# araffin/srl-zoo

Measured on AMD Instinct MI355X. Metric: images/sec (224x224x3) AE+VAE train step, higher is better.
Workload: dtype f32; 1 GPU; synthetic 224x224x3 obs, --losses autoencoder, custom_cnn, state-dim 200, bs=256 per GPU (512 frames fwd+bwd per step per GPU), Adam lr 0.005, normalised fp32 observations resident in HBM; global_batch=256, parallelism=dp1, rccl_ranks=1, devices=1

## Files before the change

### include/srlz.h

```cpp
#ifndef SRLZ_H
#define SRLZ_H

#include <stddef.h>
#include <stdint.h>

#ifdef __cplusplus
extern "C" {
#endif

typedef void* srlz_stream_t;

enum srlz_status {
  SRLZ_OK = 0,
  SRLZ_ERR_BAD_DESC = -1,
  SRLZ_ERR_WORKSPACE = -2,
  SRLZ_ERR_HIP = -3,
  SRLZ_ERR_NULL = -4
};

#define SRLZ_ABI_VERSION 104
int srlz_version(void);
const char* srlz_last_error(void);
int srlz_device_cus(void);

// ... 429 lines not shown
int srlz_beam_search(const float* states, const float* wf, const float* bf, const float* w1, const float* b1, const float* w2,
                     const float* b2, const float* w3, const float* b3, int* best_plan, float* best_return, int* leaf_plans,
                     float* leaf_returns, void* ws, size_t ws_bytes, int N, int W, int T, int S, int A, int H, int n_rewards,
                     float gamma, const float* goal, long long goal_env_stride, float goal_weight, int goal_mode,
                     srlz_stream_t stream);

int srlz_horizon_supported(int S, int A, int H, int n_rewards, int has_reward);
int srlz_horizon_rows(const float* states, const int* actions, const int* starts, const int* len, const float* wf, const float* bf,
                      const float* w1, const float* b1, const float* w2, const float* b2, const float* w3, const float* b3, float* err,
                      float* base, float* reward_logits, float* trajectory, int N, int M, int T, int S, int A, int H, int n_rewards,
                      srlz_stream_t stream);
int srlz_horizon_sums(const float* err, const float* base, const float* reward_logits, const int* labels, const int* starts,
                      const int* len, int M, int T, long long* count, double* sum_err, double* sum_base, long long* hits,
                      srlz_stream_t stream);

int srlz_conv64_debug_program(const srlz_conv64_desc* d, int backward_data, int* out, int cap);
int srlz_linear_debug_route(int op, int M, int N, int K, int Kout, const void* a, const void* b, int has_ws, size_t ws_bytes,
                            int out[3]);
int srlz_debug_mfma_peak(float* out, int blocks, int iters, srlz_stream_t stream);
int srlz_debug_mfma_valu(float* out, int blocks, int iters, int valu_per_mfma, int kind, int split, srlz_stream_t stream);
int srlz_debug_placement(unsigned* out, int blocks, int lds_bytes, int spin, srlz_stream_t stream);
int srlz_debug_conv1_fwd_generic(const float* x_nchw, const float* w_ref, float* y_nhwc, float* stats_partial,
                                 const srlz_skinny_desc* d, srlz_stream_t stream);
int srlz_debug_conv1_fwd_u8_generic(const uint8_t* x_u8, const float* norm_lut, const float* w_ref, float* y_nhwc,
                                    float* stats_partial, const srlz_skinny_desc* d, srlz_stream_t stream);
int srlz_debug_conv1_bwd_weight_fused_generic(const float* x_nchw, const float* y_nhwc, const float* bnp, const uint8_t* argmax,
                                              const float* dpooled, const float* sums, int training, float* dw_ref, void* ws,
                                              size_t ws_bytes, const srlz_skinny_desc* d, const struct srlz_pool_desc_s* pd,
                                              srlz_stream_t stream);
int srlz_debug_conv1_bwd_weight_fused_u8_generic(const uint8_t* x_u8, const float* norm_lut, const float* y_nhwc, const float* bnp,
                                                 const uint8_t* argmax, const float* dpooled, const float* sums, int training,
                                                 float* dw_ref, void* ws, size_t ws_bytes, const srlz_skinny_desc* d,
                                                 const struct srlz_pool_desc_s* pd, srlz_stream_t stream);

#ifdef __cplusplus
}
#endif
#endif
```

### srl-zoo_amd/csrc/wino.hip

```cpp
#include "common.h"

namespace {

typedef float f32x2 __attribute__((ext_vector_type(2)));
typedef unsigned u32x2 __attribute__((ext_vector_type(2)));

constexpr int WN_THREADS = 256;
constexpr int WN_TP = 32;
constexpr int WN_CHUNK = 16 * 4 * 64 * 4;
constexpr int WN_VCHUNK = 16 * 4 * WN_TP * 4;
constexpr int WN_VCOMP = 4 * WN_TP * 4;
constexpr unsigned WN_DROP = 0x80000000u;

struct WinoProg {
  int N, G;
  int H, W;
  int PA, PB;
  int ppi, ppg, tpg;
  unsigned mPPI, mPB;
  int sPPI, sPB;
  long long gstride;
};

__global__ void conv64_wino_pack_kernel(const float* __restrict__ w_ref, float* __restrict__ uf, float* __restrict__ ub) {
// ... 93 lines not shown
#pragma unroll
  for (int hv = 0; hv < 2; ++hv) {
    f32x2 e[4][2];
#pragma unroll
    for (int r = 0; r < 4; ++r) {
      if (hv == 0) {
        e[r][0] = rw.d[r * 4 + 0] - rw.d[r * 4 + 2];
        e[r][1] = rw.d[r * 4 + 1] + rw.d[r * 4 + 2];
      } else {
        e[r][0] = rw.d[r * 4 + 2] - rw.d[r * 4 + 1];
        e[r][1] = rw.d[r * 4 + 1] - rw.d[r * 4 + 3];
      }
    }
#pragma unroll
    for (int j = 0; j < 2; ++j) {
      const int nu = 2 * hv + j;
      *(f32x2*)(Vw + (0 * 4 + nu) * WN_VCOMP) = e[0][j] - e[2][j];
      *(f32x2*)(Vw + (1 * 4 + nu) * WN_VCOMP) = e[1][j] + e[2][j];
      *(f32x2*)(Vw + (2 * 4 + nu) * WN_VCOMP) = e[2][j] - e[1][j];
      *(f32x2*)(Vw + (3 * 4 + nu) * WN_VCOMP) = e[1][j] - e[3][j];
    }
    __builtin_amdgcn_sched_barrier(0);
  }
}

__device__ __forceinline__ f32x4 wn_load4(__amdgpu_buffer_rsrc_t b, unsigned voff, int soff) {
  const __attribute__((ext_vector_type(4))) unsigned v = __builtin_amdgcn_raw_buffer_load_b128(b, voff, soff, 0);
  return f32x4{__uint_as_float(v[0]), __uint_as_float(v[1]), __uint_as_float(v[2]), __uint_as_float(v[3])};
}

constexpr int WN_AQ = 4;
static_assert(64 % WN_AQ == 0, "the ring of weight operands wraps with the tile");

__device__ __forceinline__ f32x4 wn_uload(__amdgpu_buffer_rsrc_t ub, unsigned uvoff, int step, int uo) {
  const __attribute__((ext_vector_type(4))) unsigned v = __builtin_amdgcn_raw_buffer_load_b128(ub, uvoff, (step & 63) * 4096 + uo, 0);
  return f32x4{__uint_as_float(v[0]), __uint_as_float(v[1]), __uint_as_float(v[2]), __uint_as_float(v[3])};
}

template <int PH>
__device__ __forceinline__ void wn_mfma_phase(f32x4 (&acc)[16][2], f32x4 (&aq)[WN_AQ], const float* __restrict__ Bp,
                                              __amdgpu_buffer_rsrc_t ub, unsigned uvoff, int uo) {
  f32x4 b0n = *(const f32x4*)(Bp), b1n = *(const f32x4*)(Bp + 256);
#pragma unroll
  for (int comp = 0; comp < 16; ++comp) {
    const int step = PH * 16 + comp;
    const f32x4 a = aq[step % WN_AQ];
    const f32x4 b0 = b0n, b1 = b1n;
    if (comp < 15) {
      b0n = *(const f32x4*)(Bp + (comp + 1) * WN_VCOMP);
      b1n = *(const f32x4*)(Bp + (comp + 1) * WN_VCOMP + 256);
    }
#pragma unroll
    for (int i = 0; i < 4; ++i) {
      if (PH == 0 && i == 0) {
        const f32x4 z = {0.f, 0.f, 0.f, 0.f};
        acc[comp][0] = __builtin_amdgcn_mfma_f32_16x16x4f32(a[i], b0[i], z, 0, 0, 0);
        acc[comp][1] = __builtin_amdgcn_mfma_f32_16x16x4f32(a[i], b1[i], z, 0, 0, 0);
      } else {
        acc[comp][0] = __builtin_amdgcn_mfma_f32_16x16x4f32(a[i], b0[i], acc[comp][0], 0, 0, 0);
        acc[comp][1] = __builtin_amdgcn_mfma_f32_16x16x4f32(a[i], b1[i], acc[comp][1], 0, 0, 0);
      }
    }
    aq[step % WN_AQ] = wn_uload(ub, uvoff, step + WN_AQ, uo);
  }
  __builtin_amdgcn_sched_group_barrier(0x100, 2, 0);
#pragma unroll
  for (int comp = 0; comp < 16; ++comp) {
    if (comp < 15) __builtin_amdgcn_sched_group_barrier(0x100, 2, 0);
    __builtin_amdgcn_sched_group_barrier(0x008, 8, 0);
    __builtin_amdgcn_sched_group_barrier(0x020, 1, 0);
  }
  __builtin_amdgcn_sched_barrier(0);
}

__device__ __forceinline__ float wn_row16_sum(float v) {
  v += __uint_as_float(__builtin_amdgcn_update_dpp(0, __float_as_uint(v), 0x128, 0xf, 0xf, false));
  v += __uint_as_float(__builtin_amdgcn_update_dpp(0, __float_as_uint(v), 0x124, 0xf, 0xf, false));
  v += __uint_as_float(__builtin_amdgcn_update_dpp(0, __float_as_uint(v), 0x122, 0xf, 0xf, false));
  v += __uint_as_float(__builtin_amdgcn_update_dpp(0, __float_as_uint(v), 0x121, 0xf, 0xf, false));
  return v;
}

constexpr int WN_ZBLOCKS = 64;
__global__ __launch_bounds__(256) void conv64_wino_poolsum_zero_scale_kernel(const float* __restrict__ dx, const PoolSum ps, float* __restrict__ partial,
                                                                            int N, int H, int W, long long gstride, int rows, int first_row) {
  const int g = blockIdx.y;
  const float* __restrict__ rec = ps.bnp + g * 256;
  const int c4 = threadIdx.x & 15;
  const auto [mean, pinv, psc, psh] = load_bn_quads(rec, c4);
  unsigned zmask = 0;
#pragma unroll
  for (int j = 0; j < 4; ++j) zmask |= ((fabsf(psc[j]) <= 1e-3f * fabsf(psh[j]) || psc[j] == 0.f) ? 1u : 0u) << j;
  double s1[4] = {0.0, 0.0, 0.0, 0.0}, s2[4] = {0.0, 0.0, 0.0, 0.0};
  if (__syncthreads_or(zmask != 0)) {
    const long long pixels = (long long)N * H * W;
    for (long long pix = (long long)blockIdx.x * 16 + (threadIdx.x >> 4); pix < pixels; pix += (long long)gridDim.x * 16) {
      if (!zmask) continue;
      const int n = (int)(pix / (H * W));
      const int yy = (int)(pix - (long long)n * H * W) / W, xx = (int)(pix - ((long long)n * H + yy) * W);
      const uint32_t packed = *(const uint32_t*)(ps.argmax + (size_t)g * gstride + (size_t)pix * 64 + c4 * 4);
      const f32x4 v = *(const f32x4*)(dx + (size_t)g * gstride + (size_t)pix * 64 + c4 * 4);
#pragma unroll
      for (int j = 0; j < 4; ++j)
        if ((zmask >> j) & 1u) {
          const int a = (packed >> (8 * j)) & 0xff;
          const int iy = yy * 2 - ps.pad + a / 3, ix = xx * 2 - ps.pad + a % 3;
          const float vy = ps.y[g * ps.y_gstride + ((size_t)(n * ps.H + iy) * ps.W + ix) * 64 + c4 * 4 + j];
          if (vy * psc[j] + psh[j] > 0.f) {
            s1[j] += (double)v[j];
            s2[j] += (double)(v[j] * ((vy - mean[j]) * pinv[j]));
          }
        }
    }
  }
  bn_bwd_combine_store(s1, s2, partial + ((size_t)g * rows + first_row + blockIdx.x) * 128);
}

template <bool PSUM, bool FUSE>
__global__ __launch_bounds__(WN_THREADS, 2) void conv64_wino_kernel(const float* __restrict__ x_all, const float* __restrict__ upack,
                                                                    const float* __restrict__ bias, float* __restrict__ y_all,
                                                                    float* __restrict__ stats_partial, const WinoProg P, int ntiles,
                                                                    const PoolSum ps, const float* __restrict__ x_bnp) {
  extern __shared__ __attribute__((aligned(16))) unsigned char smem[];
  float* Vs = (float*)smem;
  int* ptab = (int*)(Vs + 2 * WN_VCHUNK);

  const int tid = threadIdx.x;
  int lane = tid & 63;
  asm volatile("" : "+v"(lane));
  const int wave = tid >> 6;
  const int t_pt = wave * 8 + (lane >> 3), t_cp = lane & 7;
  const int cb = wave;
  const int l15 = lane & 15, g = lane >> 4;
  float* Vw = Vs + (t_pt * 4 + ((t_cp >> 1) ^ (((t_pt >> 2) & 1) << 1))) * 4 + 2 * (t_cp & 1);
  const float* Bp = Vs + (l15 * 4 + (g ^ (((l15 >> 2) & 1) << 1))) * 4;
  const unsigned uvoff = (unsigned)(g * 64 + 16 * cb + l15) * 16u;
  const __amdgpu_buffer_rsrc_t ub = raw_buffer(upack, 4u * WN_CHUNK * 4u);

  const int xcd = blockIdx.x & 7, wi = blockIdx.x >> 3, wpx = gridDim.x >> 3;
  const int tq = ntiles >> 3, tr = ntiles & 7;
  const int tbase = (xcd < tr) ? xcd * (tq + 1) : tr * (tq + 1) + (xcd - tr) * tq;
  const int tcnt = tq + (xcd < tr ? 1 : 0);
  int k = wi;
  if (k >= tcnt) return;

  const unsigned xbytes = (unsigned)(P.gstride * 4) + (unsigned)(P.W + 1) * 256u;
  const unsigned ybytes = (unsigned)(P.gstride * 4);
  const __amdgpu_buffer_rsrc_t sbuf = raw_buffer(stats_partial, stats_partial ? (unsigned)(P.G * (P.tpg + (PSUM ? WN_ZBLOCKS : 0))) * 512u : 0u);

  WinoRaw rw;
  WinoPatch wp;
  f32x4 aq[WN_AQ];
  int parity = 0;
  {
    const int tile = tbase + k;
    const int grp = tile / P.tpg;
    const __amdgpu_buffer_rsrc_t xb = raw_buffer(x_all + grp * P.gstride - (P.W + 1) * 64, xbytes);
    wn_patch(wp, P, tile - grp * P.tpg, t_pt, t_cp, ptab + t_pt);
    const float* bnrec = FUSE ? x_bnp + grp * 256 : nullptr;
    wn_request<FUSE>(rw, wp, xb, P.W, 0, bnrec, t_cp);
    wn_land<FUSE>(rw, wp, Vw);
    wn_request<FUSE>(rw, wp, xb, P.W, 1, bnrec, t_cp);
#pragma unroll
    for (int i = 0; i < WN_AQ; ++i) aq[i] = wn_uload(ub, uvoff, i, 0);
  }
  for (; k < tcnt; k += wpx, parity ^= 1) {
    const int tile = tbase + k;
    const int grp = tile / P.tpg;
    const int til = tile - grp * P.tpg;
    const __amdgpu_buffer_rsrc_t xb = raw_buffer(x_all + grp * P.gstride - (P.W + 1) * 64, xbytes);
    const int k2 = k + wpx;
    const bool more = k2 < tcnt;
    const int tile2 = tbase + (more ? k2 : k);
    const int grp2 = tile2 / P.tpg;
    const __amdgpu_buffer_rsrc_t xb2 = raw_buffer(x_all + grp2 * P.gstride - (P.W + 1) * 64, xbytes);
    int uo = 0;
    asm volatile("" : "+s"(uo));
    f32x4 acc[16][2];
#pragma unroll
    for (int p = 0; p < 4; ++p) {
      __syncthreads();
      wn_land<FUSE>(rw, wp, Vw + ((p + 1) & 1) * WN_VCHUNK);
      if (p < 2) {
        wn_request<FUSE>(rw, wp, xb, P.W, p + 2, FUSE ? x_bnp + grp * 256 : nullptr, t_cp);
      } else {
        if (p == 2) wn_patch(wp, P, tile2 - grp2 * P.tpg, t_pt, t_cp, ptab + (parity ^ 1) * WN_TP + t_pt);
        wn_request<FUSE>(rw, wp, xb2, P.W, p - 2, FUSE ? x_bnp + grp2 * 256 : nullptr, t_cp);
      }
      __builtin_amdgcn_sched_barrier(0);
      if (p == 0) wn_mfma_phase<0>(acc, aq, Bp, ub, uvoff, uo);
      if (p == 1) wn_mfma_phase<1>(acc, aq, Bp + WN_VCHUNK, ub, uvoff, uo);
      if (p == 2) wn_mfma_phase<2>(acc, aq, Bp, ub, uvoff, uo);
      if (p == 3) wn_mfma_phase<3>(acc, aq, Bp + WN_VCHUNK, ub, uvoff, uo);
    }
    const __amdgpu_buffer_rsrc_t yb = raw_buffer(y_all + grp * P.gstride, ybytes);
    f32x4 s4 = {0.f, 0.f, 0.f, 0.f}, q4 = {0.f, 0.f, 0.f, 0.f};
    f32x4 bias4 = {0.f, 0.f, 0.f, 0.f};
    if (bias) bias4 = *(const f32x4*)(bias + 16 * cb + 4 * g);
    f32x4 pA = {0.f, 0.f, 0.f, 0.f}, pB = pA, pthr = pA;
    const __amdgpu_buffer_rsrc_t zb = raw_buffer(PSUM ? ps.pooled + grp * P.gstride : nullptr, PSUM ? ybytes : 0u);
    if constexpr (PSUM) {
      const float* __restrict__ rec = ps.bnp + grp * 256 + 16 * cb + 4 * g;
      const f32x4 mean = *(const f32x4*)rec, pinv = *(const f32x4*)(rec + 64), psc = *(const f32x4*)(rec + 128), psh = *(const f32x4*)(rec + 192);
#pragma unroll
      for (int e = 0; e < 4; ++e) {
        const bool zero = fabsf(psc[e]) <= 1e-3f * fabsf(psh[e]) || psc[e] == 0.f;
        pthr[e] = zero ? __builtin_inff() : 0.f;
        const float isc = zero ? 0.f : 1.f / psc[e];
        pA[e] = pinv[e] * isc;
        pB[e] = zero ? 0.f : -(psh[e] * isc + mean[e]) * pinv[e];
      }
    }
#pragma unroll
    for (int s = 0; s < 2; ++s) {
      const int pix = ptab[parity * WN_TP + 16 * s + l15];
      const bool ok = pix >= 0;
      const unsigned yoff = ok ? (unsigned)pix * 256u + (unsigned)(16 * cb + 4 * g) * 4u : WN_DROP;
      f32x4 z00, z01, z10, z11;
      if constexpr (PSUM) {
        z00 = wn_load4(zb, yoff, 0); z01 = wn_load4(zb, yoff, 256);
        z10 = wn_load4(zb, yoff, P.W * 256); z11 = wn_load4(zb, yoff, P.W * 256 + 256);
      }
      const f32x4 bz = {ok ? bias4[0] : 0.f, ok ? bias4[1] : 0.f, ok ? bias4[2] : 0.f, ok ? bias4[3] : 0.f};
      f32x4 y00 = bz, y01 = bz, y10 = bz, y11 = bz;
#pragma unroll
      for (int nu = 0; nu < 4; ++nu) {
        const f32x4 t0 = acc[0 + nu][s] + acc[4 + nu][s] + acc[8 + nu][s];
        const f32x4 t1 = acc[4 + nu][s] - acc[8 + nu][s] - acc[12 + nu][s];
        if (nu < 3) { y00 += t0; y10 += t1; }
        if (nu == 1) { y01 += t0; y11 += t1; }
        if (nu >= 2) { y01 -= t0; y11 -= t1; }
      }
      __builtin_amdgcn_raw_buffer_store_b128(y00, yb, yoff, 0, 0);
      __builtin_amdgcn_raw_buffer_store_b128(y01, yb, yoff, 256, 0);
      __builtin_amdgcn_raw_buffer_store_b128(y10, yb, yoff, P.W * 256, 0);
      __builtin_amdgcn_raw_buffer_store_b128(y11, yb, yoff, P.W * 256 + 256, 0);
      if constexpr (PSUM) {
#pragma unroll
        for (int e = 0; e < 4; ++e) {
          s4[e] += ((z00[e] > pthr[e] ? y00[e] : 0.f) + (z01[e] > pthr[e] ? y01[e] : 0.f)) +
                   ((z10[e] > pthr[e] ? y10[e] : 0.f) + (z11[e] > pthr[e] ? y11[e] : 0.f));
        }
        q4 += (y00 * z00 + y01 * z01) + (y10 * z10 + y11 * z11);
      } else if constexpr (FUSE) {
        const f32x4 ts = (y00 + y01) + (y10 + y11), tq = (y00 * y00 + y01 * y01) + (y10 * y10 + y11 * y11);
#pragma unroll
        for (int e = 0; e < 4; ++e) { s4[e] += ok ? ts[e] : 0.f; q4[e] += ok ? tq[e] : 0.f; }
      } else {
        s4 += (y00 + y01) + (y10 + y11);
        q4 += (y00 * y00 + y01 * y01) + (y10 * y10 + y11 * y11);
      }
      __builtin_amdgcn_sched_barrier(0);
    }
    if constexpr (PSUM) {
#pragma unroll
      for (int e = 0; e < 4; ++e) q4[e] = __builtin_fmaf(pA[e], q4[e], pB[e] * s4[e]);
    }
#pragma unroll
    for (int e = 0; e < 4; ++e) { s4[e] = wn_row16_sum(s4[e]); q4[e] = wn_row16_sum(q4[e]); }
    const unsigned rec = (unsigned)(grp * (P.tpg + (PSUM ? WN_ZBLOCKS : 0)) + til) * 512u + (unsigned)(16 * cb + 4 * g) * 4u;
    __builtin_amdgcn_raw_buffer_store_b128(s4, sbuf, l15 == 0 ? rec : WN_DROP, 0, 0);
    __builtin_amdgcn_raw_buffer_store_b128(q4, sbuf, l15 == 0 ? rec + 256u : WN_DROP, 0, 0);
  }
}

int wino_program(WinoProg* P, const srlz_conv64_desc* d) {
  if (!d || d->transposed || d->ksize != 3 || d->stride != 1 || d->pad != 1) return 1;
  if (d->hi != d->ho || d->wi != d->wo || (d->hi & 1) || (d->wi & 1) || d->hi < 4 || d->wi < 4 || d->n <= 0) return 1;
  const int G = d->groups > 1 ? d->groups : 1;
  if (d->n % G) return 1;
  P->G = G; P->N = d->n / G; P->H = d->hi; P->W = d->wi; P->PA = d->hi / 2; P->PB = d->wi / 2;
  const long long ppi = (long long)P->PA * P->PB, ppg = ppi * P->N;
  const long long gfl = (long long)P->N * P->H * P->W * 64;
  if (gfl * 4 + (long long)(P->W + 1) * 256 >= 0x7FFF0000LL || ppg + WN_TP >= (1LL << 31) || ppi < 2) return 1;
  P->ppi = (int)ppi; P->ppg = (int)ppg; P->tpg = (int)((ppg + WN_TP - 1) / WN_TP);
  P->gstride = gfl;
  fastdiv_init((unsigned)P->ppi, &P->mPPI, &P->sPPI);
  fastdiv_init((unsigned)P->PB, &P->mPB, &P->sPB);
  return 0;
}

constexpr int WG_SP = 8;
constexpr int WG_OP = 8 * WG_SP * 64;
constexpr int WG_COMP = WG_SP * 64;

struct WinoWgradRaw { f32x2 d[12]; f32x2 g[4]; };

struct WinoWgradProg {
  int N, H, W, PA, PB, ppi;
  int total;
  int stages;
  int spw;
  unsigned mPPI, mPB;
  int sPPI, sPB;
};

// ... 232 lines not shown
  P->stages = (int)((total + WG_SP - 1) / WG_SP);
  P->mPPI = F.mPPI; P->sPPI = F.sPPI; P->mPB = F.mPB; P->sPB = F.sPB;
  int g = 2 * srlz_device_cus();
  g = (g + 15) & ~15;
  while (g > 16 && (g >> 1) * 4 > P->stages) g -= 16;
  const int slices = g >> 1;
  P->spw = (P->stages + slices - 1) / slices;
  *grid = g;
  return 0;
}

}

extern "C" int srlz_conv64_wino_supported(const srlz_conv64_desc* d) {
  WinoProg P;
  return wino_program(&P, d) ? 0 : 1;
}

extern "C" size_t srlz_conv64_wino_packed_floats(void) { return (size_t)4 * WN_CHUNK; }

extern "C" int srlz_conv64_wino_pack_weights(const float* w_ref, float* upack_fwd, float* upack_bwd, srlz_stream_t stream) {
  SRLZ_REQUIRE(w_ref && (upack_fwd || upack_bwd), SRLZ_ERR_NULL, "conv64_wino_pack_weights: null pointer");
  SRLZ_LAUNCH(conv64_wino_pack_kernel, dim3(16), dim3(256), 0, as_stream(stream), w_ref, upack_fwd, upack_bwd);
  return 0;
}

extern "C" int srlz_conv64_wino_tiles(const srlz_conv64_desc* d) {
  WinoProg P;
  if (wino_program(&P, d)) return -1;
  return P.G * P.tpg;
}

static int wino_launch(const float* x, const float* upack, const float* bias, float* y, float* partial, const WinoProg& P,
                       const PoolSum* ps, const float* x_bnp, srlz_stream_t stream) {
  const int ntiles = P.G * P.tpg;
  int grid = 2 * srlz_device_cus();
  if (ntiles < grid) grid = ntiles;
  grid = (grid + 7) & ~7;
  const size_t lds = (size_t)2 * WN_VCHUNK * 4 + 2 * WN_TP * 4;
  const PoolSum none = SRLZ_NO_POOLSUM;
  hipStream_t st = as_stream(stream);
  if (ps) {
    SRLZ_MAX_LDS((conv64_wino_kernel<true, false>), lds);
    SRLZ_LAUNCH((conv64_wino_kernel<true, false>), dim3(grid), dim3(WN_THREADS), lds, st, x, upack, bias, y, partial, P, ntiles, *ps, x_bnp);
  } else if (x_bnp) {
    SRLZ_MAX_LDS((conv64_wino_kernel<false, true>), lds);
    SRLZ_LAUNCH((conv64_wino_kernel<false, true>), dim3(grid), dim3(WN_THREADS), lds, st, x, upack, bias, y, partial, P, ntiles, none, x_bnp);
  } else {
    SRLZ_MAX_LDS((conv64_wino_kernel<false, false>), lds);
    SRLZ_LAUNCH((conv64_wino_kernel<false, false>), dim3(grid), dim3(WN_THREADS), lds, st, x, upack, bias, y, partial, P, ntiles, none, x_bnp);
  }
  if (ps) {
    SRLZ_LAUNCH(conv64_wino_poolsum_zero_scale_kernel, dim3(WN_ZBLOCKS, P.G), dim3(256), 0, st, (const float*)y, *ps, partial, P.N, P.H,
                P.W, P.gstride, P.tpg + WN_ZBLOCKS, P.tpg);
  }
  return 0;
}

extern "C" int srlz_conv64_wino_bwd_data_rows(const srlz_conv64_desc* d) {
  WinoProg P;
  if (wino_program(&P, d)) return -1;
  return P.G * (P.tpg + WN_ZBLOCKS);
}

extern "C" int srlz_conv64_wino_fwd(const float* x, const float* upack, const float* bias, float* y, float* stats_partial,
                                    const float* x_bnp, const srlz_conv64_desc* d, srlz_stream_t stream) {
  SRLZ_REQUIRE(x && upack && y, SRLZ_ERR_NULL, "conv64_wino_fwd: null pointer");
  WinoProg P;
  SRLZ_REQUIRE(wino_program(&P, d) == 0, SRLZ_ERR_BAD_DESC,
               "conv64_wino_fwd: 3x3 stride 1 pad 1 on even sizes only (ask srlz_conv64_wino_supported)");
  return wino_launch(x, upack, bias, y, stats_partial, P, nullptr, x_bnp, stream);
}

extern "C" int srlz_conv64_wino_bwd_data(const float* dy, const float* upack_bwd, float* dx, const srlz_conv64_desc* d, srlz_stream_t stream) {
  SRLZ_REQUIRE(dy && upack_bwd && dx, SRLZ_ERR_NULL, "conv64_wino_bwd_data: null pointer");
  WinoProg P;
  SRLZ_REQUIRE(wino_program(&P, d) == 0, SRLZ_ERR_BAD_DESC,
               "conv64_wino_bwd_data: 3x3 stride 1 pad 1 on even sizes only (ask srlz_conv64_wino_supported)");
  return wino_launch(dy, upack_bwd, nullptr, dx, nullptr, P, nullptr, nullptr, stream);
}

extern "C" int srlz_conv64_wino_bwd_data_pool_sums(const float* dy, const float* upack_bwd, float* dx, const float* pooled,
                                                   const float* pool_bnp, const float* pool_y, const uint8_t* pool_argmax,
                                                   const srlz_pool_desc* pd, float* bn_bwd_partial, const srlz_conv64_desc* d,
                                                   srlz_stream_t stream) {
  SRLZ_REQUIRE(dy && upack_bwd && dx && pooled && pool_bnp && pool_y && pool_argmax && pd && bn_bwd_partial, SRLZ_ERR_NULL,
               "conv64_wino_bwd_data_pool_sums: null pointer");
  WinoProg P;
  SRLZ_REQUIRE(wino_program(&P, d) == 0, SRLZ_ERR_BAD_DESC,
               "conv64_wino_bwd_data_pool_sums: 3x3 stride 1 pad 1 on even sizes only (ask srlz_conv64_wino_supported)");
  SRLZ_REQUIRE(pd->n == d->n && pd->hp == d->hi && pd->wp == d->wi && !pd->out_nchw && (pd->groups > 1 ? pd->groups : 1) == P.G,
               SRLZ_ERR_BAD_DESC, "conv64_wino_bwd_data_pool_sums: the pooled map [%d,%d,%d] is not this layer's input [%d,%d,%d]", pd->n, pd->hp,
               pd->wp, d->n, d->hi, d->wi);
  const PoolSum ps = {pooled, pool_bnp, pool_y, pool_argmax, (long long)(pd->n / P.G) * pd->h * pd->w * 64, pd->h, pd->w, pd->pool_pad};
  return wino_launch(dy, upack_bwd, nullptr, dx, bn_bwd_partial, P, &ps, nullptr, stream);
}

extern "C" size_t srlz_conv64_wino_bwd_weight_workspace(const srlz_conv64_desc* d) {
  WinoWgradProg P;
  int grid;
  if (wino_wgrad_program(&P, d, &grid)) return 0;
  return (size_t)grid * 8 * 4096 * sizeof(float) + (size_t)WG_CHUNKS * 16 * 4096 * sizeof(double);
}

extern "C" int srlz_conv64_wino_bwd_weight(const float* x, const float* dy, float* dw_ref, void* ws, size_t ws_bytes,
                                           const srlz_conv64_desc* d, srlz_stream_t stream) {
  SRLZ_REQUIRE(x && dy && dw_ref && ws, SRLZ_ERR_NULL, "conv64_wino_bwd_weight: null pointer");
  WinoWgradProg P;
  int grid;
  SRLZ_REQUIRE(wino_wgrad_program(&P, d, &grid) == 0, SRLZ_ERR_BAD_DESC,
               "conv64_wino_bwd_weight: 3x3 stride 1 pad 1 on even sizes only (ask srlz_conv64_wino_supported)");
  const size_t part_bytes = (size_t)grid * 8 * 4096 * sizeof(float);
  SRLZ_REQUIRE(ws_bytes >= part_bytes + (size_t)WG_CHUNKS * 16 * 4096 * sizeof(double), SRLZ_ERR_WORKSPACE,
               "conv64_wino_bwd_weight: workspace too small (%zu bytes)", ws_bytes);
  hipStream_t st = as_stream(stream);
  const size_t lds = (size_t)4 * WG_OP * 4;
  SRLZ_MAX_LDS(conv64_wino_wgrad_kernel, lds);
  SRLZ_LAUNCH(conv64_wino_wgrad_kernel, dim3(grid), dim3(256), lds, st, x, dy, (float*)ws, P);
  double* mid = (double*)((char*)ws + part_bytes);
  const int npair = grid >> 1, per = (npair + WG_CHUNKS - 1) / WG_CHUNKS;
  SRLZ_LAUNCH(conv64_wino_wgrad_reduce_a, dim3(65536 / 256, WG_CHUNKS), dim3(256), 0, st, (const float*)ws, mid, grid, per);
  SRLZ_LAUNCH(conv64_wino_wgrad_reduce_b, dim3(256), dim3(256), 0, st, (const double*)mid, WG_CHUNKS, dw_ref);
  return 0;
}
```

### srl-zoo_amd/srlz/_cabi.py

```python
import ctypes
import os
from ctypes import c_int, c_longlong, c_ulonglong, c_float, c_double, c_void_p, c_size_t, c_char_p, POINTER, Structure

_HERE = os.path.dirname(os.path.abspath(__file__))
LIB_PATH = os.path.join(_HERE, "libsrlz_hip.so")


ABI_VERSION = 104


class SrlzError(RuntimeError):
    pass


class Conv64Desc(Structure):
    _fields_ = [("n", c_int), ("hi", c_int), ("wi", c_int), ("ho", c_int), ("wo", c_int), ("ksize", c_int),
                ("stride", c_int), ("pad", c_int), ("transposed", c_int), ("groups", c_int)]


class SkinnyDesc(Structure):
    _fields_ = [("n", c_int), ("c", c_int), ("himg", c_int), ("wimg", c_int), ("hf", c_int), ("wf", c_int),
                ("kind", c_int), ("groups", c_int)]


# ... 47 lines not shown
_ID = POINTER(InferDecDesc)

_PROTOS = {
    "srlz_version": (c_int, []),
    "srlz_last_error": (c_char_p, []),
    "srlz_device_cus": (c_int, []),
    "srlz_conv64_packed_floats": (c_size_t, []),
    "srlz_conv64_pack_weights": (c_int, [P, P, P, _C64, P]),
    "srlz_conv64_fwd_tiles": (c_int, [_C64]),
    "srlz_conv64_fwd": (c_int, [P, P, P, P, P, P, _C64, P]),
    "srlz_conv64_bwd_data": (c_int, [P, P, P, _BO, _C64, P]),
    "srlz_conv64_bwd_weight_workspace": (c_size_t, [_C64]),
    "srlz_conv64_bwd_fused_supported": (c_int, [_C64]),
    "srlz_conv64_gather_pipe_supported": (c_int, [_C64, c_int]),
    "srlz_conv64_scatter_pipe_supported": (c_int, [_C64, c_int]),
    "srlz_conv64_bwd_fused_workspace": (c_size_t, [_C64]),
    "srlz_conv64_bwd_fused": (c_int, [P, P, P, _BO, P, P, P, P, P, P, c_size_t, _C64, P]),
    "srlz_conv64_bwd_fused_bn_rows": (c_int, [_C64]),
    "srlz_conv64_wino_supported": (c_int, [_C64]),
    "srlz_conv64_wino_packed_floats": (c_size_t, []),
    "srlz_conv64_wino_pack_weights": (c_int, [P, P, P, P]),
    "srlz_conv64_wino_tiles": (c_int, [_C64]),
    "srlz_conv64_wino_fwd": (c_int, [P, P, P, P, P, P, _C64, P]),
    "srlz_conv64_wino_bwd_data": (c_int, [P, P, P, _C64, P]),
    "srlz_conv64_wino_bwd_weight_workspace": (c_size_t, [_C64]),
    "srlz_conv64_wino_bwd_weight": (c_int, [P, P, P, P, c_size_t, _C64, P]),
    "srlz_conv64_wino_bwd_data_rows": (c_int, [_C64]),
    "srlz_conv64_wino_bwd_data_pool_sums": (c_int, [P, P, P, P, P, P, P, _PD, P, _C64, P]),
    "srlz_conv64_bwd_weight": (c_int, [P, P, P, P, P, _BO, P, c_size_t, _C64, P]),
    "srlz_conv64_bwd_weight_plan": (c_int, [_C64, c_int, c_int, POINTER(c_int)]),
    "srlz_conv64_bwd_fused_workgroups": (c_int, [_C64]),
    "srlz_conv1_workgroups": (c_int, [_SK]),
    "srlz_conv1_buffer_staging_supported": (c_int, [_SK]),
    "srlz_debug_conv1_fwd_generic": (c_int, [P, P, P, P, _SK, P]),
    "srlz_debug_conv1_fwd_u8_generic": (c_int, [P, P, P, P, P, _SK, P]),
    "srlz_debug_conv1_bwd_weight_fused_generic": (c_int, [P, P, P, P, P, P, c_int, P, P, c_size_t, _SK, _PD, P]),
    "srlz_debug_conv1_bwd_weight_fused_u8_generic": (c_int, [P, P, P, P, P, P, P, c_int, P, P, c_size_t, _SK, _PD, P]),
    "srlz_convT_out_os_plan": (c_int, [_SK, c_int, POINTER(c_int)]),
    "srlz_conv64_debug_program": (c_int, [_C64, c_int, POINTER(c_int), c_int]),
    "srlz_linear_debug_route": (c_int, [c_int, c_int, c_int, c_int, c_int, P, P, c_int, c_size_t, POINTER(c_int)]),
    "srlz_debug_placement": (c_int, [P, c_int, c_int, c_int, P]),
    "srlz_debug_mfma_peak": (c_int, [P, c_int, c_int, P]),
    "srlz_debug_mfma_valu": (c_int, [P, c_int, c_int, c_int, c_int, c_int, P]),
    "srlz_convn_packed_floats": (c_size_t, [_CN]),
    "srlz_convn_pack_weights": (c_int, [P, P, _CN, P]),
    "srlz_convn_fwd_tiles": (c_int, [_CN]),
    "srlz_convn_fwd": (c_int, [P, P, P, P, P, _CN, P]),
    "srlz_bn_finalize_chunks_workspace": (c_size_t, [c_int, c_int]),
    "srlz_bn_finalize_chunks": (c_int, [P, c_int, c_int, c_int, c_longlong, P, P, c_float, c_float, P, P, P, P, P, c_size_t, P]),
    "srlz_bn_eval_params_chunks": (c_int, [P, P, P, P, c_float, c_int, P, P]),
    "srlz_bn_add_relu": (c_int, [P, P, P, P, P, c_longlong, c_int, c_int, P]),
    "srlz_avgpool_nhwc": (c_int, [P, P, c_int, c_int, c_int, P]),
    "srlz_prelu_fwd": (c_int, [P, P, P, c_longlong, P]),
    "srlz_prelu_bwd": (c_int, [P, P, P, P, P, c_longlong, P]),
    "srlz_triplet_fwd": (c_int, [P, P, P, c_int, c_int, c_float, P, P, P]),
    "srlz_triplet_bwd": (c_int, [P, P, P, P, P, c_int, c_int, P, P, P, P]),
    "srlz_skinny_tiles": (c_int, [_SK]),
    "srlz_conv64_bwd_data_tiles": (c_int, [_C64]),
    "srlz_conv64_bwd_data_pool_sums": (c_int, [P, P, P, P, P, P, P, _PD, P, _C64, P]),
    "srlz_conv1_fwd": (c_int, [P, P, P, P, _SK, P]),
    "srlz_conv1_fwd_u8": (c_int, [P, P, P, P, P, _SK, P]),
    "srlz_conv1_bwd_weight_fused_u8": (c_int, [P, P, P, P, P, P, P, c_int, P, P, c_size_t, _SK, _PD, P]),
    "srlz_convT_out_fwd_loss_u8": (c_int, [P, P, P, P, P, P, P, P, P, _SK, P]),
    "srlz_normalize_lut": (c_int, [P, P]),
    "srlz_normalize_u8_planar": (c_int, [P, P, P, c_int, c_int, c_longlong, P]),
    "srlz_copy_frames_u8": (c_int, [P, P, c_longlong, P, P, c_longlong, c_int, c_longlong, P]),
# ... 222 lines not shown
```

Before: 45890 images/s.

## Fold Winograd output transform into last MFMA phase of pooled data-gradient kernel

For the pooled-sum backward-data Winograd kernel, the last matrix phase now visits components column by column and applies the output transform for each column as soon as it completes. The pooled-map loads are issued mid-phase, so the transform arithmetic and memory latency overlap the remaining MFMAs instead of running in a serial epilogue. Per-group BN pool parameters are now computed once into LDS rather than per tile. The old epilogue path stays reachable through a debug entry point, at the cost of extra LDS and register pressure in the folded kernel.

```diff
diff --git a/include/srlz.h b/include/srlz.h
--- a/include/srlz.h
+++ b/include/srlz.h
@@ -485,6 +485,10 @@
                                                  const uint8_t* argmax, const float* dpooled, const float* sums, int training,
                                                  float* dw_ref, void* ws, size_t ws_bytes, const srlz_skinny_desc* d,
                                                  const struct srlz_pool_desc_s* pd, srlz_stream_t stream);
+int srlz_debug_conv64_wino_bwd_data_pool_sums_parent(const float* dy, const float* upack_bwd, float* dx, const float* pooled,
+                                                     const float* pool_bnp, const float* pool_y, const uint8_t* pool_argmax,
+                                                     const struct srlz_pool_desc_s* pd, float* bn_bwd_partial,
+                                                     const srlz_conv64_desc* d, srlz_stream_t stream);
 
 #ifdef __cplusplus
 }
diff --git a/srl-zoo_amd/csrc/wino.hip b/srl-zoo_amd/csrc/wino.hip
--- a/srl-zoo_amd/csrc/wino.hip
+++ b/srl-zoo_amd/csrc/wino.hip
@@ -149,44 +149,92 @@
 constexpr int WN_AQ = 4;
 static_assert(64 % WN_AQ == 0, "the ring of weight operands wraps with the tile");
 
+template <bool FOLD>
+__device__ __forceinline__ constexpr int wn_comp(int ph, int i) { return (FOLD && ph == 3) ? 4 * (i & 3) + (i >> 2) : i; }
+template <bool FOLD>
+__device__ __forceinline__ constexpr int wn_step(int q) { return (q & 63) < 48 ? (q & 63) : 48 + wn_comp<FOLD>(3, q & 15); }
+
 __device__ __forceinline__ f32x4 wn_uload(__amdgpu_buffer_rsrc_t ub, unsigned uvoff, int step, int uo) {
   const __attribute__((ext_vector_type(4))) unsigned v = __builtin_amdgcn_raw_buffer_load_b128(ub, uvoff, (step & 63) * 4096 + uo, 0);
   return f32x4{__uint_as_float(v[0]), __uint_as_float(v[1]), __uint_as_float(v[2]), __uint_as_float(v[3])};
 }
 
-template <int PH>
+struct WinoFold {
+  f32x4 y[2][4];
+  f32x4 z[2][4];
+  unsigned yoff[2];
+  __amdgpu_buffer_rsrc_t zb;
+  int wrow;
+};
+
+__device__ __forceinline__ void wn_zrequest(WinoFold& f, int s) {
+  f.z[s][0] = wn_load4(f.zb, f.yoff[s], 0);
+  f.z[s][1] = wn_load4(f.zb, f.yoff[s], 256);
+  f.z[s][2] = wn_load4(f.zb, f.yoff[s], f.wrow);
+  f.z[s][3] = wn_load4(f.zb, f.yoff[s], f.wrow + 256);
+}
+
+template <int NU>
+__device__ __forceinline__ void wn_fold_column(const f32x4 (&acc)[16][2], WinoFold& f) {
+#pragma unroll
+  for (int s = 0; s < 2; ++s) {
+    const f32x4 t0 = acc[0 + NU][s] + acc[4 + NU][s] + acc[8 + NU][s];
+    const f32x4 t1 = acc[4 + NU][s] - acc[8 + NU][s] - acc[12 + NU][s];
+    if (NU < 3) { f.y[s][0] += t0; f.y[s][2] += t1; }
+    if (NU == 1) { f.y[s][1] += t0; f.y[s][3] += t1; }
+    if (NU >= 2) { f.y[s][1] -= t0; f.y[s][3] -= t1; }
+  }
+}
+
+template <int PH, bool FOLD = false>
 __device__ __forceinline__ void wn_mfma_phase(f32x4 (&acc)[16][2], f32x4 (&aq)[WN_AQ], const float* __restrict__ Bp,
-                                              __amdgpu_buffer_rsrc_t ub, unsigned uvoff, int uo) {
+                                              __amdgpu_buffer_rsrc_t ub, unsigned uvoff, int uo, WinoFold* fo = nullptr) {
+  constexpr bool CM = FOLD && PH == 3;
   f32x4 b0n = *(const f32x4*)(Bp), b1n = *(const f32x4*)(Bp + 256);
 #pragma unroll
-  for (int comp = 0; comp < 16; ++comp) {
-    const int step = PH * 16 + comp;
-    const f32x4 a = aq[step % WN_AQ];
+  for (int i = 0; i < 16; ++i) {
+    const int q = PH * 16 + i, comp = wn_comp<FOLD>(PH, i);
+    const f32x4 a = aq[q % WN_AQ];
     const f32x4 b0 = b0n, b1 = b1n;
-    if (comp < 15) {
-      b0n = *(const f32x4*)(Bp + (comp + 1) * WN_VCOMP);
-      b1n = *(const f32x4*)(Bp + (comp + 1) * WN_VCOMP + 256);
-    }
-#pragma unroll
-    for (int i = 0; i < 4; ++i) {
-      if (PH == 0 && i == 0) {
+    if (i < 15) {
+      b0n = *(const f32x4*)(Bp + wn_comp<FOLD>(PH, i + 1) * WN_VCOMP);
+      b1n = *(const f32x4*)(Bp + wn_comp<FOLD>(PH, i + 1) * WN_VCOMP + 256);
+    }
+#pragma unroll
+    for (int k = 0; k < 4; ++k) {
+      if (PH == 0 && k == 0) {
         const f32x4 z = {0.f, 0.f, 0.f, 0.f};
-        acc[comp][0] = __builtin_amdgcn_mfma_f32_16x16x4f32(a[i], b0[i], z, 0, 0, 0);
-        acc[comp][1] = __builtin_amdgcn_mfma_f32_16x16x4f32(a[i], b1[i], z, 0, 0, 0);
+        acc[comp][0] = __builtin_amdgcn_mfma_f32_16x16x4f32(a[k], b0[k], z, 0, 0, 0);
+        acc[comp][1] = __builtin_amdgcn_mfma_f32_16x16x4f32(a[k], b1[k], z, 0, 0, 0);
       } else {
-        acc[comp][0] = __builtin_amdgcn_mfma_f32_16x16x4f32(a[i], b0[i], acc[comp][0], 0, 0, 0);
-        acc[comp][1] = __builtin_amdgcn_mfma_f32_16x16x4f32(a[i], b1[i], acc[comp][1], 0, 0, 0);
-      }
-    }
-    aq[step % WN_AQ] = wn_uload(ub, uvoff, step + WN_AQ, uo);
+        acc[comp][0] = __builtin_amdgcn_mfma_f32_16x16x4f32(a[k], b0[k], acc[comp][0], 0, 0, 0);
+        acc[comp][1] = __builtin_amdgcn_mfma_f32_16x16x4f32(a[k], b1[k], acc[comp][1], 0, 0, 0);
+      }
+    }
+    aq[q % WN_AQ] = wn_uload(ub, uvoff, wn_step<FOLD>(q + WN_AQ), uo);
+    if constexpr (CM) {
+      if (i == 3) wn_fold_column<0>(acc, *fo);
+      if (i == 7) {
+        wn_fold_column<1>(acc, *fo);
+        wn_zrequest(*fo, 0);
+        wn_zrequest(*fo, 1);
+      }
+      if (i == 11) wn_fold_column<2>(acc, *fo);
+      if (i == 15) wn_fold_column<3>(acc, *fo);
+    }
   }
   __builtin_amdgcn_sched_group_barrier(0x100, 2, 0);
 #pragma unroll
-  for (int comp = 0; comp < 16; ++comp) {
-    if (comp < 15) __builtin_amdgcn_sched_group_barrier(0x100, 2, 0);
+  for (int i = 0; i < 16; ++i) {
+    if (i < 15) __builtin_amdgcn_sched_group_barrier(0x100, 2, 0);
     __builtin_amdgcn_sched_group_barrier(0x008, 8, 0);
     __builtin_amdgcn_sched_group_barrier(0x020, 1, 0);
-  }
+    if constexpr (CM) {
+      if (i == 4 || i == 8 || i == 12) __builtin_amdgcn_sched_group_barrier(0x002, 64, 0);
+      if (i == 8) __builtin_amdgcn_sched_group_barrier(0x020, 8, 0);
+    }
+  }
+  if constexpr (CM) __builtin_amdgcn_sched_group_barrier(0x002, 64, 0);
   __builtin_amdgcn_sched_barrier(0);
 }
 
@@ -233,14 +281,15 @@
   bn_bwd_combine_store(s1, s2, partial + ((size_t)g * rows + first_row + blockIdx.x) * 128);
 }
 
-template <bool PSUM, bool FUSE>
-__global__ __launch_bounds__(WN_THREADS, 2) void conv64_wino_kernel(const float* __restrict__ x_all, const float* __restrict__ upack,
-                                                                    const float* __restrict__ bias, float* __restrict__ y_all,
-                                                                    float* __restrict__ stats_partial, const WinoProg P, int ntiles,
-                                                                    const PoolSum ps, const float* __restrict__ x_bnp) {
+template <bool PSUM, bool FUSE, bool FOLD>
+__device__ __forceinline__ void wn_tiles(const float* __restrict__ x_all, const float* __restrict__ upack, const float* __restrict__ bias,
+                                         float* __restrict__ y_all, float* __restrict__ stats_partial, const WinoProg P, int ntiles,
+                                         const PoolSum ps, const float* __restrict__ x_bnp) {
+  static_assert(!FOLD || (PSUM && !FUSE), "the fold inside the matrix phase is the pooled-block data gradient's");
   extern __shared__ __attribute__((aligned(16))) unsigned char smem[];
   float* Vs = (float*)smem;
   int* ptab = (int*)(Vs + 2 * WN_VCHUNK);
+  float* pprm = (float*)(ptab + 2 * WN_TP);
 
   const int tid = threadIdx.x;
   int lane = tid & 63;
@@ -268,7 +317,7 @@
   WinoRaw rw;
   WinoPatch wp;
   f32x4 aq[WN_AQ];
-  int parity = 0;
+  int parity = 0, pgrp = -1;
   {
     const int tile = tbase + k;
     const int grp = tile / P.tpg;
@@ -294,6 +343,7 @@
     int uo = 0;
     asm volatile("" : "+s"(uo));
     f32x4 acc[16][2];
+    WinoFold fo;
 #pragma unroll
     for (int p = 0; p < 4; ++p) {
       __syncthreads();
@@ -304,11 +354,36 @@
         if (p == 2) wn_patch(wp, P, tile2 - grp2 * P.tpg, t_pt, t_cp, ptab + (parity ^ 1) * WN_TP + t_pt);
         wn_request<FUSE>(rw, wp, xb2, P.W, p - 2, FUSE ? x_bnp + grp2 * 256 : nullptr, t_cp);
       }
+      if constexpr (FOLD) {
+        if (p == 0 && grp != pgrp) {
+          pgrp = grp;
+          if (tid < 64) {
+            const float* __restrict__ rec = ps.bnp + grp * 256 + tid;
+            const float mean = rec[0], pinv = rec[64], psc = rec[128], psh = rec[192];
+            const bool zero = fabsf(psc) <= 1e-3f * fabsf(psh) || psc == 0.f;
+            const float isc = zero ? 0.f : 1.f / psc;
+            pprm[tid] = pinv * isc;
+            pprm[64 + tid] = zero ? 0.f : -__builtin_fmaf(psh, isc, mean) * pinv;
+            pprm[128 + tid] = zero ? __builtin_inff() : 0.f;
+          }
+        }
+        if (p == 3) {
+          fo.zb = raw_buffer(ps.pooled + grp * P.gstride, (unsigned)(P.gstride * 4));
+          fo.wrow = P.W * 256;
+#pragma unroll
+          for (int s = 0; s < 2; ++s) {
+            const int pix = ptab[parity * WN_TP + 16 * s + l15];
+            fo.yoff[s] = pix >= 0 ? (unsigned)pix * 256u + (unsigned)(16 * cb + 4 * g) * 4u : WN_DROP;
+#pragma unroll
+            for (int j = 0; j < 4; ++j) fo.y[s][j] = f32x4{0.f, 0.f, 0.f, 0.f};
+          }
+        }
+      }
       __builtin_amdgcn_sched_barrier(0);
-      if (p == 0) wn_mfma_phase<0>(acc, aq, Bp, ub, uvoff, uo);
-      if (p == 1) wn_mfma_phase<1>(acc, aq, Bp + WN_VCHUNK, ub, uvoff, uo);
-      if (p == 2) wn_mfma_phase<2>(acc, aq, Bp, ub, uvoff, uo);
-      if (p == 3) wn_mfma_phase<3>(acc, aq, Bp + WN_VCHUNK, ub, uvoff, uo);
+      if (p == 0) wn_mfma_phase<0, FOLD>(acc, aq, Bp, ub, uvoff, uo);
+      if (p == 1) wn_mfma_phase<1, FOLD>(acc, aq, Bp + WN_VCHUNK, ub, uvoff, uo);
+      if (p == 2) wn_mfma_phase<2, FOLD>(acc, aq, Bp, ub, uvoff, uo);
+      if (p == 3) wn_mfma_phase<3, FOLD>(acc, aq, Bp + WN_VCHUNK, ub, uvoff, uo, &fo);
     }
     const __amdgpu_buffer_rsrc_t yb = raw_buffer(y_all + grp * P.gstride, ybytes);
     f32x4 s4 = {0.f, 0.f, 0.f, 0.f}, q4 = {0.f, 0.f, 0.f, 0.f};
@@ -316,58 +391,82 @@
     if (bias) bias4 = *(const f32x4*)(bias + 16 * cb + 4 * g);
     f32x4 pA = {0.f, 0.f, 0.f, 0.f}, pB = pA, pthr = pA;
     const __amdgpu_buffer_rsrc_t zb = raw_buffer(PSUM ? ps.pooled + grp * P.gstride : nullptr, PSUM ? ybytes : 0u);
-    if constexpr (PSUM) {
-      const float* __restrict__ rec = ps.bnp + grp * 256 + 16 * cb + 4 * g;
-      const f32x4 mean = *(const f32x4*)rec, pinv = *(const f32x4*)(rec + 64), psc = *(const f32x4*)(rec + 128), psh = *(const f32x4*)(rec + 192);
-#pragma unroll
-      for (int e = 0; e < 4; ++e) {
-        const bool zero = fabsf(psc[e]) <= 1e-3f * fabsf(psh[e]) || psc[e] == 0.f;
-        pthr[e] = zero ? __builtin_inff() : 0.f;
-        const float isc = zero ? 0.f : 1.f / psc[e];
-        pA[e] = pinv[e] * isc;
-        pB[e] = zero ? 0.f : -(psh[e] * isc + mean[e]) * pinv[e];
-      }
-    }
-#pragma unroll
-    for (int s = 0; s < 2; ++s) {
-      const int pix = ptab[parity * WN_TP + 16 * s + l15];
-      const bool ok = pix >= 0;
-      const unsigned yoff = ok ? (unsigned)pix * 256u + (unsigned)(16 * cb + 4 * g) * 4u : WN_DROP;
-      f32x4 z00, z01, z10, z11;
+    if constexpr (FOLD) {
+#pragma unroll
+      for (int s = 0; s < 2; ++s) {
+        __builtin_amdgcn_raw_buffer_store_b128(fo.y[s][0], yb, fo.yoff[s], 0, 0);
+        __builtin_amdgcn_raw_buffer_store_b128(fo.y[s][1], yb, fo.yoff[s], 256, 0);
+        __builtin_amdgcn_raw_buffer_store_b128(fo.y[s][2], yb, fo.yoff[s], P.W * 256, 0);
+        __builtin_amdgcn_raw_buffer_store_b128(fo.y[s][3], yb, fo.yoff[s], P.W * 256 + 256, 0);
+      }
+      pA = *(const f32x4*)(pprm + 16 * cb + 4 * g);
+      pB = *(const f32x4*)(pprm + 64 + 16 * cb + 4 * g);
+      pthr = *(const f32x4*)(pprm + 128 + 16 * cb + 4 * g);
+#pragma unroll
+      for (int s = 0; s < 2; ++s) {
+        const f32x4(&y)[4] = fo.y[s];
+        const f32x4(&z)[4] = fo.z[s];
+#pragma unroll
+        for (int e = 0; e < 4; ++e) {
+          s4[e] += ((z[0][e] > pthr[e] ? y[0][e] : 0.f) + (z[1][e] > pthr[e] ? y[1][e] : 0.f)) +
+                   ((z[2][e] > pthr[e] ? y[2][e] : 0.f) + (z[3][e] > pthr[e] ? y[3][e] : 0.f));
+          q4[e] += __builtin_fmaf(y[0][e], z[0][e], y[1][e] * z[1][e]) + __builtin_fmaf(y[2][e], z[2][e], y[3][e] * z[3][e]);
+        }
+      }
+    } else {
       if constexpr (PSUM) {
-        z00 = wn_load4(zb, yoff, 0); z01 = wn_load4(zb, yoff, 256);
-        z10 = wn_load4(zb, yoff, P.W * 256); z11 = wn_load4(zb, yoff, P.W * 256 + 256);
-      }
-      const f32x4 bz = {ok ? bias4[0] : 0.f, ok ? bias4[1] : 0.f, ok ? bias4[2] : 0.f, ok ? bias4[3] : 0.f};
-      f32x4 y00 = bz, y01 = bz, y10 = bz, y11 = bz;
-#pragma unroll
-      for (int nu = 0; nu < 4; ++nu) {
-        const f32x4 t0 = acc[0 + nu][s] + acc[4 + nu][s] + acc[8 + nu][s];
-        const f32x4 t1 = acc[4 + nu][s] - acc[8 + nu][s] - acc[12 + nu][s];
-        if (nu < 3) { y00 += t0; y10 += t1; }
-        if (nu == 1) { y01 += t0; y11 += t1; }
-        if (nu >= 2) { y01 -= t0; y11 -= t1; }
-      }
-      __builtin_amdgcn_raw_buffer_store_b128(y00, yb, yoff, 0, 0);
-      __builtin_amdgcn_raw_buffer_store_b128(y01, yb, yoff, 256, 0);
-      __builtin_amdgcn_raw_buffer_store_b128(y10, yb, yoff, P.W * 256, 0);
-      __builtin_amdgcn_raw_buffer_store_b128(y11, yb, yoff, P.W * 256 + 256, 0);
-      if constexpr (PSUM) {
+        const float* __restrict__ rec = ps.bnp + grp * 256 + 16 * cb + 4 * g;
+        const f32x4 mean = *(const f32x4*)rec, pinv = *(const f32x4*)(rec + 64), psc = *(const f32x4*)(rec + 128), psh = *(const f32x4*)(rec + 192);
 #pragma unroll
         for (int e = 0; e < 4; ++e) {
-          s4[e] += ((z00[e] > pthr[e] ? y00[e] : 0.f) + (z01[e] > pthr[e] ? y01[e] : 0.f)) +
-                   ((z10[e] > pthr[e] ? y10[e] : 0.f) + (z11[e] > pthr[e] ? y11[e] : 0.f));
+          const bool zero = fabsf(psc[e]) <= 1e-3f * fabsf(psh[e]) || psc[e] == 0.f;
+          pthr[e] = zero ? __builtin_inff() : 0.f;
+          const float isc = zero ? 0.f : 1.f / psc[e];
+          pA[e] = pinv[e] * isc;
+          pB[e] = zero ? 0.f : -(psh[e] * isc + mean[e]) * pinv[e];
         }
-        q4 += (y00 * z00 + y01 * z01) + (y10 * z10 + y11 * z11);
-      } else if constexpr (FUSE) {
-        const f32x4 ts = (y00 + y01) + (y10 + y11), tq = (y00 * y00 + y01 * y01) + (y10 * y10 + y11 * y11);
-#pragma unroll
-        for (int e = 0; e < 4; ++e) { s4[e] += ok ? ts[e] : 0.f; q4[e] += ok ? tq[e] : 0.f; }
-      } else {
-        s4 += (y00 + y01) + (y10 + y11);
-        q4 += (y00 * y00 + y01 * y01) + (y10 * y10 + y11 * y11);
-      }
-      __builtin_amdgcn_sched_barrier(0);
+      }
+#pragma unroll
+      for (int s = 0; s < 2; ++s) {
+        const int pix = ptab[parity * WN_TP + 16 * s + l15];
+        const bool ok = pix >= 0;
+        const unsigned yoff = ok ? (unsigned)pix * 256u + (unsigned)(16 * cb + 4 * g) * 4u : WN_DROP;
+        f32x4 z00, z01, z10, z11;
+        if constexpr (PSUM) {
+          z00 = wn_load4(zb, yoff, 0); z01 = wn_load4(zb, yoff, 256);
+          z10 = wn_load4(zb, yoff, P.W * 256); z11 = wn_load4(zb, yoff, P.W * 256 + 256);
+        }
+        const f32x4 bz = {ok ? bias4[0] : 0.f, ok ? bias4[1] : 0.f, ok ? bias4[2] : 0.f, ok ? bias4[3] : 0.f};
+        f32x4 y00 = bz, y01 = bz, y10 = bz, y11 = bz;
+#pragma unroll
+        for (int nu = 0; nu < 4; ++nu) {
+          const f32x4 t0 = acc[0 + nu][s] + acc[4 + nu][s] + acc[8 + nu][s];
+          const f32x4 t1 = acc[4 + nu][s] - acc[8 + nu][s] - acc[12 + nu][s];
+          if (nu < 3) { y00 += t0; y10 += t1; }
+          if (nu == 1) { y01 += t0; y11 += t1; }
+          if (nu >= 2) { y01 -= t0; y11 -= t1; }
+        }
+        __builtin_amdgcn_raw_buffer_store_b128(y00, yb, yoff, 0, 0);
+        __builtin_amdgcn_raw_buffer_store_b128(y01, yb, yoff, 256, 0);
+        __builtin_amdgcn_raw_buffer_store_b128(y10, yb, yoff, P.W * 256, 0);
+        __builtin_amdgcn_raw_buffer_store_b128(y11, yb, yoff, P.W * 256 + 256, 0);
+        if constexpr (PSUM) {
+#pragma unroll
+          for (int e = 0; e < 4; ++e) {
+            s4[e] += ((z00[e] > pthr[e] ? y00[e] : 0.f) + (z01[e] > pthr[e] ? y01[e] : 0.f)) +
+                     ((z10[e] > pthr[e] ? y10[e] : 0.f) + (z11[e] > pthr[e] ? y11[e] : 0.f));
+          }
+          q4 += (y00 * z00 + y01 * z01) + (y10 * z10 + y11 * z11);
+        } else if constexpr (FUSE) {
+          const f32x4 ts = (y00 + y01) + (y10 + y11), tq = (y00 * y00 + y01 * y01) + (y10 * y10 + y11 * y11);
+#pragma unroll
+          for (int e = 0; e < 4; ++e) { s4[e] += ok ? ts[e] : 0.f; q4[e] += ok ? tq[e] : 0.f; }
+        } else {
+          s4 += (y00 + y01) + (y10 + y11);
+          q4 += (y00 * y00 + y01 * y01) + (y10 * y10 + y11 * y11);
+        }
+        __builtin_amdgcn_sched_barrier(0);
+      }
     }
     if constexpr (PSUM) {
 #pragma unroll
@@ -379,6 +478,21 @@
     __builtin_amdgcn_raw_buffer_store_b128(s4, sbuf, l15 == 0 ? rec : WN_DROP, 0, 0);
     __builtin_amdgcn_raw_buffer_store_b128(q4, sbuf, l15 == 0 ? rec + 256u : WN_DROP, 0, 0);
   }
+}
+
+template <bool PSUM, bool FUSE>
+__global__ __launch_bounds__(WN_THREADS, 2) void conv64_wino_kernel(const float* __restrict__ x_all, const float* __restrict__ upack,
+                                                                    const float* __restrict__ bias, float* __restrict__ y_all,
+                                                                    float* __restrict__ stats_partial, const WinoProg P, int ntiles,
+                                                                    const PoolSum ps, const float* __restrict__ x_bnp) {
+  wn_tiles<PSUM, FUSE, PSUM>(x_all, upack, bias, y_all, stats_partial, P, ntiles, ps, x_bnp);
+}
+
+__global__ __launch_bounds__(WN_THREADS, 2) void conv64_wino_poolsum_parent_kernel(const float* __restrict__ x_all, const float* __restrict__ upack,
+                                                                                   const float* __restrict__ bias, float* __restrict__ y_all,
+                                                                                   float* __restrict__ stats_partial, const WinoProg P, int ntiles,
+                                                                                   const PoolSum ps, const float* __restrict__ x_bnp) {
+  wn_tiles<true, false, false>(x_all, upack, bias, y_all, stats_partial, P, ntiles, ps, x_bnp);
 }
 
 int wino_program(WinoProg* P, const srlz_conv64_desc* d) {
@@ -677,15 +791,18 @@
 }
 
 static int wino_launch(const float* x, const float* upack, const float* bias, float* y, float* partial, const WinoProg& P,
-                       const PoolSum* ps, const float* x_bnp, srlz_stream_t stream) {
+                       const PoolSum* ps, const float* x_bnp, srlz_stream_t stream, bool parent = false) {
   const int ntiles = P.G * P.tpg;
   int grid = 2 * srlz_device_cus();
   if (ntiles < grid) grid = ntiles;
   grid = (grid + 7) & ~7;
-  const size_t lds = (size_t)2 * WN_VCHUNK * 4 + 2 * WN_TP * 4;
+  const size_t lds = (size_t)2 * WN_VCHUNK * 4 + 2 * WN_TP * 4 + 3 * 64 * 4;
   const PoolSum none = SRLZ_NO_POOLSUM;
   hipStream_t st = as_stream(stream);
-  if (ps) {
+  if (ps && parent) {
+    SRLZ_MAX_LDS(conv64_wino_poolsum_parent_kernel, lds);
+    SRLZ_LAUNCH(conv64_wino_poolsum_parent_kernel, dim3(grid), dim3(WN_THREADS), lds, st, x, upack, bias, y, partial, P, ntiles, *ps, x_bnp);
+  } else if (ps) {
     SRLZ_MAX_LDS((conv64_wino_kernel<true, false>), lds);
     SRLZ_LAUNCH((conv64_wino_kernel<true, false>), dim3(grid), dim3(WN_THREADS), lds, st, x, upack, bias, y, partial, P, ntiles, *ps, x_bnp);
   } else if (x_bnp) {
@@ -725,10 +842,9 @@
   return wino_launch(dy, upack_bwd, nullptr, dx, nullptr, P, nullptr, nullptr, stream);
 }
 
-extern "C" int srlz_conv64_wino_bwd_data_pool_sums(const float* dy, const float* upack_bwd, float* dx, const float* pooled,
-                                                   const float* pool_bnp, const float* pool_y, const uint8_t* pool_argmax,
-                                                   const srlz_pool_desc* pd, float* bn_bwd_partial, const srlz_conv64_desc* d,
-                                                   srlz_stream_t stream) {
+static int wino_bwd_data_pool_sums(const float* dy, const float* upack_bwd, float* dx, const float* pooled, const float* pool_bnp,
+                                   const float* pool_y, const uint8_t* pool_argmax, const srlz_pool_desc* pd, float* bn_bwd_partial,
+                                   const srlz_conv64_desc* d, srlz_stream_t stream, bool parent) {
   SRLZ_REQUIRE(dy && upack_bwd && dx && pooled && pool_bnp && pool_y && pool_argmax && pd && bn_bwd_partial, SRLZ_ERR_NULL,
                "conv64_wino_bwd_data_pool_sums: null pointer");
   WinoProg P;
@@ -738,7 +854,21 @@
                SRLZ_ERR_BAD_DESC, "conv64_wino_bwd_data_pool_sums: the pooled map [%d,%d,%d] is not this layer's input [%d,%d,%d]", pd->n, pd->hp,
                pd->wp, d->n, d->hi, d->wi);
   const PoolSum ps = {pooled, pool_bnp, pool_y, pool_argmax, (long long)(pd->n / P.G) * pd->h * pd->w * 64, pd->h, pd->w, pd->pool_pad};
-  return wino_launch(dy, upack_bwd, nullptr, dx, bn_bwd_partial, P, &ps, nullptr, stream);
+  return wino_launch(dy, upack_bwd, nullptr, dx, bn_bwd_partial, P, &ps, nullptr, stream, parent);
+}
+
+extern "C" int srlz_conv64_wino_bwd_data_pool_sums(const float* dy, const float* upack_bwd, float* dx, const float* pooled,
+                                                   const float* pool_bnp, const float* pool_y, const uint8_t* pool_argmax,
+                                                   const srlz_pool_desc* pd, float* bn_bwd_partial, const srlz_conv64_desc* d,
+                                                   srlz_stream_t stream) {
+  return wino_bwd_data_pool_sums(dy, upack_bwd, dx, pooled, pool_bnp, pool_y, pool_argmax, pd, bn_bwd_partial, d, stream, false);
+}
+
+extern "C" int srlz_debug_conv64_wino_bwd_data_pool_sums_parent(const float* dy, const float* upack_bwd, float* dx, const float* pooled,
+                                                                const float* pool_bnp, const float* pool_y, const uint8_t* pool_argmax,
+                                                                const srlz_pool_desc* pd, float* bn_bwd_partial,
+                                                                const srlz_conv64_desc* d, srlz_stream_t stream) {
+  return wino_bwd_data_pool_sums(dy, upack_bwd, dx, pooled, pool_bnp, pool_y, pool_argmax, pd, bn_bwd_partial, d, stream, true);
 }
 
 extern "C" size_t srlz_conv64_wino_bwd_weight_workspace(const srlz_conv64_desc* d) {
diff --git a/srl-zoo_amd/srlz/_cabi.py b/srl-zoo_amd/srlz/_cabi.py
--- a/srl-zoo_amd/srlz/_cabi.py
+++ b/srl-zoo_amd/srlz/_cabi.py
@@ -103,6 +103,7 @@
     "srlz_conv64_bwd_fused_workgroups": (c_int, [_C64]),
     "srlz_conv1_workgroups": (c_int, [_SK]),
     "srlz_conv1_buffer_staging_supported": (c_int, [_SK]),
+    "srlz_debug_conv64_wino_bwd_data_pool_sums_parent": (c_int, [P, P, P, P, P, P, P, _PD, P, _C64, P]),
     "srlz_debug_conv1_fwd_generic": (c_int, [P, P, P, P, _SK, P]),
     "srlz_debug_conv1_fwd_u8_generic": (c_int, [P, P, P, P, P, _SK, P]),
     "srlz_debug_conv1_bwd_weight_fused_generic": (c_int, [P, P, P, P, P, P, c_int, P, P, c_size_t, _SK, _PD, P]),
```

Result: no change. 46060 images/s, median of 6 (+0.4%).
